# LANL-Bioinformatics/KWAGE

Measured on AMD Instinct MI355X. Metric: G k-mer·sample bit-tests/sec (+ achieved HBM GB/s of the gather kernel in `roofline`), higher is better.
Workload: dtype u32

## Files before the change

kwage_amd/csrc/engine.hip:

```cpp
#include <hip/hip_runtime.h>
#include <hip/hip_ext.h>

#include <algorithm>
#include <chrono>
#include <cmath>
#include <cstdio>
#include <cctype>
#include <cstring>
#include <new>
#include <string>
#include <thread>
#include <vector>

#include <unistd.h>

#include "host.hpp"
#include "engine_state.hpp"
#include "kernels.hpp"

using namespace kwage;


struct TuningName { const char *name; int64_t Tuning::*field; };
static const TuningName TUNING_NAMES[] = {
// ... 51 lines not shown

__global__ __launch_bounds__(256) void remap_rows_kernel(uint32_t *rows, const uint64_t *pos_off, const uint32_t *nkmer, uint32_t num_hash,
                                                         const uint32_t *map, uint32_t map_len, unsigned long long *missing, uint32_t wgs_per_query)
{
	const uint32_t q = blockIdx.x / wgs_per_query, part = blockIdx.x % wgs_per_query;
	uint32_t *rq = rows + pos_off[q]*num_hash;
	const uint64_t n = (uint64_t)nkmer[q]*num_hash;
	for(uint64_t e = (uint64_t)part*blockDim.x + threadIdx.x; e < n; e += (uint64_t)wgs_per_query*blockDim.x){
		const uint32_t r = rq[e];
		uint32_t lo = 0, hi = map_len;
		while(lo < hi){
			const uint32_t mid = lo + (hi - lo)/2;
			if(map[mid] < r){ lo = mid + 1; } else { hi = mid; }
		}
		if(lo < map_len && map[lo] == r){ rq[e] = lo; }
		else{ rq[e] = 0; atomicAdd(missing, 1ull); }
	}
}

__global__ __launch_bounds__(SEARCH_THREADS) void and_refine_emit_kernel(SearchArgs a, RefineArgs ra)
{
	constexpr int B = 4;
	__shared__ WaveHitBuf hit_bufs[SEARCH_THREADS/WAVE];
	WaveHitBuf *hbuf = &hit_bufs[threadIdx.x >> 6];
	WaveHitState hst;
	const uint32_t lane = threadIdx.x & (WAVE - 1), l = lane & 7u, g = lane >> 3;
	const uint32_t n_clusters = refine_list_end(ra, 0);
	const uint32_t gw = __builtin_amdgcn_readfirstlane(blockIdx.x*(blockDim.x/WAVE) + (threadIdx.x >> 6));
	const uint32_t nw = gridDim.x*(blockDim.x/WAVE);
	for(uint64_t c0 = gw; c0 < n_clusters; c0 += (uint64_t)B*nw){
		RefineCluster cl[B];
		u32x4 m[B];
#pragma unroll
		for(int k = 0; k < B; ++k){
			const uint64_t ci = c0 + (uint64_t)k*nw;
			cl[k].q = REFINE_NONE;
			if(ci < n_clusters){ cl[k] = ra.clusters[ci]; }
		}
#pragma unroll
		for(int k = 0; k < B; ++k){
			const uint32_t groups = cl[k].kstep_groups & 0xFFu;
			m[k] = (u32x4)(0u);
			if(cl[k].q != REFINE_NONE && ((groups >> g) & 1u)){
				const uint32_t it = cl[k].first_item + __popc(groups & ((1u << g) - 1u));
				m[k] = reinterpret_cast<const u32x4*>(ra.masks)[(uint64_t)it*8 + l];
			}
		}
#pragma unroll
		for(int k = 0; k < B; ++k){
			if(cl[k].q == REFINE_NONE){ continue; }
			const uint32_t kstep = cl[k].kstep_groups >> 8;
			emit_masked_hits_buffered(a, hbuf, hst, cl[k].q, kstep*WAVE + lane, m[k], cl[k].n, (uint64_t)cl[k].q*a.runs_per_query + kstep);
		}
	}
	wave_hits_flush(a, hbuf, hst);
}

__global__ __launch_bounds__(256) void band_bucket_kernel(const uint32_t *__restrict__ rows, const uint64_t *__restrict__ pos_off, const uint32_t *__restrict__ nkmer,
                                                         uint32_t num_hash, uint32_t bands, uint32_t rows_per_band, uint32_t *__restrict__ loc, uint32_t *__restrict__ rows2)
{
// ... 407 lines not shown
template <int PLANES>
int launch_count_combine(const SearchArgs &a, uint32_t seg_planes, hipStream_t s, const StageEvents &ge)
{
	const size_t lds = (size_t)(COMBINE_WAVES/2)*PLANES*WAVE*16;
	if(lds > 48*1024){
		HIP_TRY(hipFuncSetAttribute((const void*)count_combine_kernel<PLANES>, hipFuncAttributeMaxDynamicSharedMemorySize, (int)lds));
	}
	KW_GATHER_LAUNCH(ge, false, true, (count_combine_kernel<PLANES>), dim3((a.units_per_row + WAVE - 1)/WAVE, a.n_queries), dim3(COMBINE_WAVES*WAVE), lds, s, a, seg_planes);
	return KWAGE_OK;
}

uint64_t max_segments(const SearchArgs &a, uint64_t max_segs) { return (a.n_queries > 65535) ? 1 : max_segs; }

int reserve_zeroed(DevBuf &buf, uint64_t bytes, hipStream_t s)
{
	if(bytes <= buf.cap){ return KWAGE_OK; }
	int rc = buf.reserve(bytes);
	if(rc){ return rc; }
	HIP_TRY(hipMemsetAsync(buf.p, 0, buf.cap, s));
	return KWAGE_OK;
}

int refine_setup(Slot *sl, const Tuning &tn, const SearchArgs &a, uint64_t total_rows, uint64_t max_rows, uint32_t max_seg, uint64_t item_bytes, uint64_t unit_bytes,
                 uint64_t tiles, uint64_t screen_waves, uint64_t ncu, hipStream_t gs, RefineSetup *out,
                 uint64_t exact_clusters = 0, uint64_t exact_items = 0, uint64_t exact_units = 0)
{
	int rc;
	RefineArgs &ra = out->ra;
	ra.seg_rows = (uint32_t)std::min<int64_t>(std::max<int64_t>(tn.refine_seg_rows, 8), max_seg);
	ra.seg_rows = (uint32_t)std::max<uint64_t>(ra.seg_rows, (max_rows + 65535)/65536);
	ra.min_rows = (uint32_t)std::max<int64_t>(tn.refine_min_rows, 1);
	ra.max_groups = (uint32_t)std::min<int64_t>(std::max<int64_t>(tn.refine_max_groups, 0), 16);
	uint64_t items = std::min<uint64_t>(std::max<uint64_t>(8ull*a.n_queries, 1u << 16), 1u << 20);
	items = std::max<uint64_t>(std::min<uint64_t>(items, (256ull << 20)/item_bytes), 1024);
	uint64_t units = std::min<uint64_t>(std::max<uint64_t>(32*total_rows/ra.seg_rows, 1u << 18), 1u << 25);
	if(unit_bytes){ units = std::max<uint64_t>(std::min<uint64_t>(units, (512ull << 20)/unit_bytes), 4096); }
	if(tn.refine_list_cap > 0){ items = units = (uint64_t)std::min<int64_t>(tn.refine_list_cap, 1 << 20); }
	uint64_t clusters = items;
	if(exact_units){ clusters = exact_clusters; items = exact_items; units = exact_units; }
	if(exact_units && tn.refine_list_cap > 0){ clusters = items = units = (uint64_t)std::min<int64_t>(tn.refine_list_cap, 1 << 20); }
	const uint64_t tiles_per_wave = (tiles + screen_waves - 1)/std::max<uint64_t>(screen_waves, 1);
	auto list = [&](uint64_t cap, uint64_t stat_max, uint64_t chunk_max) {
		RefineList ls;
		ls.cap = (uint32_t)cap;
		ls.stat = (tn.refine_static && !exact_units) ? (uint32_t)std::min<uint64_t>(stat_max, cap/2/std::max<uint64_t>(screen_waves, 1)) : 0u;
		ls.base = (uint32_t)(ls.stat*screen_waves);
		ls.chunk = exact_units ? 1u : (uint32_t)std::max<uint64_t>(1, std::min<uint64_t>(chunk_max, tiles_per_wave/4));
		return ls;
	};
	ra.lc = list(clusters, 32, 32);
	ra.li = list(items, 64, 64);
	ra.lu = list(units, 256, 256);
	if((rc = sl->ref_counters.reserve(8*sizeof(uint32_t)))){ return rc; }
	if((rc = sl->ref_clusters.reserve(clusters*sizeof(RefineCluster)))){ return rc; }
	if((rc = sl->ref_masks.reserve(items*item_bytes))){ return rc; }
	if((rc = sl->ref_units.reserve(units*sizeof(RefineUnit)))){ return rc; }
	if(unit_bytes && (rc = sl->ref_slab.reserve(units*unit_bytes))){ return rc; }
	ra.counters = (uint32_t*)sl->ref_counters.p;
	ra.clusters = (RefineCluster*)sl->ref_clusters.p;
	ra.masks = (uint32_t*)sl->ref_masks.p;
	ra.units = (RefineUnit*)sl->ref_units.p;
	ra.slab = (uint32_t*)sl->ref_slab.p;
	HIP_TRY(hipMemsetAsync(ra.counters, 0, 8*sizeof(uint32_t), gs));
	sl->ref_base[0] = ra.lc.base; sl->ref_base[1] = ra.li.base; sl->ref_base[2] = ra.lu.base;
	sl->ref_cap[0] = ra.lc.cap; sl->ref_cap[1] = ra.li.cap; sl->ref_cap[2] = ra.lu.cap;
	ra.queue_batch = (uint32_t)std::max<uint64_t>(1, std::min<uint64_t>(16, tiles/(8*std::max<uint64_t>(screen_waves, 1))));
	ra.check_every = (tn.count_screen_check == 16 || tn.count_screen_check == 32 || tn.count_screen_check == 64) ? (uint32_t)tn.count_screen_check : 8u;
	out->refine_wgs = (uint32_t)(ncu*8);
	out->emit_wgs = (uint32_t)(ncu*4);
	return KWAGE_OK;
}

uint32_t count_screen_blocks_per_cu(uint32_t planes, uint32_t nh)
{
	static int cache[3][5] = {};
	const int pi = (planes <= 7) ? 0 : (planes <= 10) ? 1 : 2, ni = (int)std::min(std::max(nh, 1u), 5u) - 1;
	if(cache[pi][ni] == 0){
		int nb = 0;
		hipError_t e = hipErrorUnknown;
#define KWAGE_OCC_NH(P, N) case N: e = hipOccupancyMaxActiveBlocksPerMultiprocessor(&nb, count_screen_kernel<P, N>, SEARCH_THREADS, 0); break;
#define KWAGE_OCC_P(I, P) case I: switch(ni + 1){ KWAGE_OCC_NH(P, 1) KWAGE_OCC_NH(P, 2) KWAGE_OCC_NH(P, 3) KWAGE_OCC_NH(P, 4) default: KWAGE_OCC_NH(P, 5) } break;
		switch(pi){ KWAGE_OCC_P(0, 7) KWAGE_OCC_P(1, 10) default: KWAGE_OCC_P(2, 14) }
#undef KWAGE_OCC_P
#undef KWAGE_OCC_NH
		if(e != hipSuccess || nb <= 0){ (void)hipGetLastError(); nb = 2; }
		cache[pi][ni] = nb;
// ... 39 lines not shown
			const uint32_t G = (a.units_per_row <= 4) ? 16 : (a.units_per_row <= 8) ? 8 : (a.units_per_row <= 16) ? 4 : 2;
			const uint64_t waves = ((uint64_t)a.n_queries + G - 1)/G;
			const dim3 grid((uint32_t)((waves + 3)/4)), block(SEARCH_THREADS);
			const int unroll = (waves < ncu*16) ? 16 : 8;
			snprintf(sl->kernel_name, sizeof(sl->kernel_name), "and_narrow_kernel<%u,%d>", G, unroll);
#define KWAGE_NARROW_CASE(GG) case GG: \
				if(unroll == 16){ KW_GATHER_LAUNCH(ge, true, true, (and_narrow_kernel<GG, 16>), grid, block, 0, gs, a); } \
				else{ KW_GATHER_LAUNCH(ge, true, true, (and_narrow_kernel<GG, 8>), grid, block, 0, gs, a); } break;
			switch(G){
				KWAGE_NARROW_CASE(16) KWAGE_NARROW_CASE(8) KWAGE_NARROW_CASE(4)
				default: KWAGE_NARROW_CASE(2)
			}
#undef KWAGE_NARROW_CASE
			HIP_TRY(hipGetLastError());
			return KWAGE_OK;
		}
		if(a.early_exit && tn.ee_refine && a.units_per_row >= WAVE && tn.force_segs <= 0){
			RefineSetup rs;
			const int vec = (a.units_per_row >= 4*WAVE) ? 2 : 1;
			a.segs = 1;
			a.chunks = (a.units_per_row + WAVE*vec - 1)/(WAVE*vec);
			const uint64_t tiles = (uint64_t)a.n_queries*a.chunks;
			const uint64_t screen_waves = (std::min<uint64_t>(tiles, ncu*(uint64_t)std::max<int64_t>(tn.screen_wpc, 1)) + 3)/4*4;
			if((rc = refine_setup(sl, tn, a, L->total_pos*a.num_hash, L->max_pos*a.num_hash, 1u << 20, 128, 0, tiles, screen_waves, ncu, gs, &rs))){ return rc; }
			const int unroll = (tn.refine_unroll == 16) ? 16 : 8;
			snprintf(sl->kernel_name, sizeof(sl->kernel_name), "and_screen_kernel<%d,8>+refine<%d>", vec, unroll);
			const dim3 grid((uint32_t)(screen_waves/4)), block(SEARCH_THREADS);
			if(vec == 2){ KW_GATHER_LAUNCH(ge, true, false, (and_screen_kernel<2, 8>), grid, block, 0, gs, a, rs.ra); }
			else{ KW_GATHER_LAUNCH(ge, true, false, (and_screen_kernel<1, 8>), grid, block, 0, gs, a, rs.ra); }
			if(unroll == 16){ KW_GATHER_LAUNCH(ge, false, false, (and_refine_kernel<16>), dim3(rs.refine_wgs), block, 0, gs, a, rs.ra); }
			else{ KW_GATHER_LAUNCH(ge, false, false, (and_refine_kernel<8>), dim3(rs.refine_wgs), block, 0, gs, a, rs.ra); }
			KW_GATHER_LAUNCH(ge, false, true, and_refine_emit_kernel, dim3(rs.emit_wgs), block, 0, gs, a, rs.ra);
			HIP_TRY(hipGetLastError());
			return KWAGE_OK;
		}
		const int walk_knob = (int)tn.walk;
		const uint64_t walk_min_rows = (tn.walk_min_rows >= 0) ? (uint64_t)tn.walk_min_rows : (uint64_t)WALK_MIN_ROWS_PER_WAVE*256*WALK_WAVES_PER_CU;
		const uint32_t kib = (a.units_per_row + WAVE - 1)/WAVE;
		const uint32_t walk_max_kib = (uint32_t)std::max<int64_t>(tn.walk_max_kib, 0);
		const uint32_t walk_tile = (uint32_t)std::min<int64_t>(std::max<int64_t>(tn.walk_tile_kib, 1), 16);
		const uint32_t coltiles = (kib + walk_tile - 1)/walk_tile, walk_ch = (kib + coltiles - 1)/coltiles;
		const bool walk_ee_ok = !a.early_exit;
		const uint64_t walk_slots = (uint64_t)coltiles*L->total_pos;
		const uint32_t walk_min_kib = (uint32_t)std::max<int64_t>(tn.walk_min_kib, 1);
		const int walk_unroll = (walk_ch <= 2) ? 8 : 4;
		if(walk_knob && walk_ee_ok && kib >= walk_min_kib && kib <= walk_max_kib && walk_slots*a.num_hash >= walk_min_rows && walk_slots > 0){
			const uint64_t chip_waves = ncu*WALK_WAVES_PER_CU;
// ... 80 lines not shown
			HIP_TRY(hipMemsetAsync(sl->partial.p, 0xFF, bytes, gs));
			a.partial = (uint32_t*)sl->partial.p;
		}
		snprintf(sl->kernel_name, sizeof(sl->kernel_name), "and_kernel<%d,8,nt>%s", cfg.vec, a.segs > 1 ? "+segments" : "");
		launch_and_v(a, gs, cfg, ge);
		if(a.segs > 1){
			KW_GATHER_LAUNCH(ge, false, true, and_combine_kernel, dim3((a.units_per_row + 255)/256, a.n_queries), dim3(256), 0, gs, a);
		}
	}
	else{
		a.chunks = (a.units_per_row + WAVE - 1)/WAVE;
		const uint32_t planes = planes_for(L->max_pos);
		const bool narrow = tn.narrow && a.units_per_row <= 32 && a.units_per_row > 8 && a.n_queries >= 64 && planes <= 14;
		if(a.early_exit && tn.ee_refine && !narrow && tn.force_segs <= 0 && a.units_per_row >= WAVE
		   && (uint64_t)a.n_queries*a.chunks >= (uint64_t)std::max<int64_t>(tn.count_screen_min_tiles, 1) && planes <= 14){
			const uint64_t tiles = (uint64_t)a.n_queries*a.chunks;
			uint32_t seg = (uint32_t)std::min<int64_t>(std::max<int64_t>(tn.refine_seg_rows, 8), 120)/8*8;
			int up = 7;
			if(L->max_pos > 8192){ seg = (uint32_t)((L->max_pos + 127)/128 + 7)/8*8; up = 14; }
			const uint64_t wpc = std::min<uint64_t>((uint64_t)std::max<int64_t>(tn.count_screen_wpc, 1), 4ull*count_screen_blocks_per_cu(planes, std::min(a.num_hash, 5u)));
			const uint64_t screen_waves = (std::min<uint64_t>(tiles, ncu*wpc) + 3)/4*4;
			if((rc = check_refine_units(planes, up))){ return rc; }
			RefineSetup rs;
			if((rc = refine_setup(sl, tn, a, L->total_pos, 0, seg, (uint64_t)planes*128, (uint64_t)up*128, tiles, screen_waves, ncu, gs, &rs))){ return rc; }
			rs.ra.seg_rows = seg;
			a.segs = 1;
			snprintf(sl->kernel_name, sizeof(sl->kernel_name), "count_screen_kernel<%u,%u>+refine<%d>", planes, std::min(a.num_hash, 5u), up);
			const dim3 grid((uint32_t)(screen_waves/4)), block(SEARCH_THREADS);
#define KWAGE_CS_NH(P, N) case N: KW_GATHER_LAUNCH(ge, true, false, (count_screen_kernel<P, N>), grid, block, 0, gs, a, rs.ra); break;
#define KWAGE_CS_P(P) case P: switch(std::min(a.num_hash, 5u)){ KWAGE_CS_NH(P, 1) KWAGE_CS_NH(P, 2) KWAGE_CS_NH(P, 3) KWAGE_CS_NH(P, 4) default: KWAGE_CS_NH(P, 5) } break;
			switch(planes){ KWAGE_CS_P(7) KWAGE_CS_P(10) default: KWAGE_CS_P(14) }
#undef KWAGE_CS_P
#undef KWAGE_CS_NH
			launch_count_refine_and_emit(planes, up, a, rs, gs, ge);
			HIP_TRY(hipGetLastError());
			return KWAGE_OK;
		}
		if(a.early_exit && tn.ee_refine && tn.count_trunc && tn.count_walk && !narrow && tn.force_segs <= 0 && a.units_per_row >= WAVE && L->total_pos > 0){
			const uint32_t nq = a.n_queries;
			const uint32_t tplanes = std::max<uint32_t>(planes, 10);
			const double col = std::min(1.0, std::max(0.0, g->density_max) + 3.0*std::sqrt(0.25/4096.0));
			const double pm = std::min(0.9, std::max(0.0005, std::pow(col, (double)a.num_hash)));
			static const bool trunc_debug = getenv("KWAGE_TRUNC_DEBUG") != nullptr;
			if(trunc_debug){ fprintf(stderr, "[kwage_amd] truncated count walk: sampled density %.5f, densest column %.5f, per-k-mer match probability planned with %.5f\n", g->density, g->density_max, pm); }
			if((rc = sl->trunc_host.reserve(((uint64_t)nq + 1)*sizeof(uint64_t) + (uint64_t)nq*sizeof(uint32_t)))){ return rc; }
			uint64_t *h_soff = (uint64_t*)sl->trunc_host.p;
			uint32_t *h_kcut = (uint32_t*)(h_soff + nq + 1);
// ... 16 lines not shown
				max_rest = std::max(max_rest, npos - kc);
				rest_total += npos - kc;
			}
			const uint64_t slots = (uint64_t)a.chunks*walked;
			const uint64_t chip_waves = ncu*(uint64_t)std::max<int64_t>(tn.count_walk_wpc, 1);
			const uint64_t min_rows = (tn.count_walk_min_rows >= 0) ? (uint64_t)tn.count_walk_min_rows : (uint64_t)WALK_MIN_ROWS_PER_WAVE*chip_waves;
			uint64_t seg = (uint64_t)std::min<int64_t>(std::max<int64_t>(tn.refine_seg_rows, 8), 120)/8*8;
			seg = std::max<uint64_t>(seg, ((max_rest + 127)/128 + 7)/8*8);
			const int up = (seg <= 120) ? 7 : 14;
			uint64_t units_worst = 0;
			for(uint32_t i = 0; i < nq && seg; ++i){
				const uint64_t rest = (L->h_pos_off[i + 1] - L->h_pos_off[i]) - h_kcut[i];
				units_worst += (uint64_t)a.chunks*8*((rest + seg - 1)/seg);
			}
			const uint64_t tiles = (uint64_t)nq*a.chunks;
			const uint64_t units_cap = std::max<uint64_t>(4096, std::min<uint64_t>(units_worst, (1ull << 30)/((uint64_t)up*128 + sizeof(RefineUnit))));
			if(walked*10 <= L->total_pos*7 && slots*a.num_hash >= min_rows && seg <= 16376 && rest_total > 0 && tiles*8*(uint64_t)tplanes*128 <= (1ull << 30)){
				const uint64_t want_waves = (tn.count_walk_waves > 0) ? std::min<uint64_t>((uint64_t)tn.count_walk_waves, slots)
					: std::max<uint64_t>(1, std::min<uint64_t>(chip_waves, slots*a.num_hash/WALK_MIN_ROWS_PER_WAVE));
				const WalkShape shape = walk_shape(tn, want_waves, ncu);
				const uint64_t waves = (uint64_t)shape.wgs*shape.wg_waves;
				if((rc = check_refine_units(tplanes, up))){ return rc; }
				RefineSetup rs;
				if((rc = refine_setup(sl, tn, a, rest_total, 0, (uint32_t)seg, (uint64_t)tplanes*128, (uint64_t)up*128, tiles, waves, ncu, gs, &rs, tiles, tiles*8, units_cap))){ return rc; }
				rs.ra.seg_rows = (uint32_t)seg;
				if((rc = sl->trunc_dev.reserve(((uint64_t)nq + 1)*sizeof(uint64_t) + (uint64_t)nq*sizeof(uint32_t)))){ return rc; }
				HIP_TRY(hipMemcpyAsync(sl->trunc_dev.p, sl->trunc_host.p, ((uint64_t)nq + 1)*sizeof(uint64_t) + (uint64_t)nq*sizeof(uint32_t), hipMemcpyHostToDevice, gs));
				CountWalkArgs wa;
				wa.total_slots = slots;
				wa.per_wave = (slots + waves - 1)/waves;
				wa.coltiles = a.chunks;
				if((rc = sl->cwalk_slab.reserve(waves*2*tplanes*1024))){ return rc; }
				if((rc = reserve_zeroed(sl->cwalk_arrived, waves*CWALK_LEVELS*sizeof(uint32_t), gs))){ return rc; }
				wa.slab = (uint32_t*)sl->cwalk_slab.p;
				wa.arrived = (uint32_t*)sl->cwalk_arrived.p;
				wa.slot_off = (const uint64_t*)sl->trunc_dev.p;
				wa.kcut = (const uint32_t*)((const uint64_t*)sl->trunc_dev.p + nq + 1);
				a.segs = 1;
				snprintf(sl->kernel_name, sizeof(sl->kernel_name), "count_walk_kernel<%u,%u,trunc>+refine<%d>", tplanes, std::min(a.num_hash, 5u), up);
				launch_count_walk_planes<true>(tplanes, a, wa, rs.ra, shape, gs, ge);
				launch_count_refine_and_emit(tplanes, up, a, rs, gs, ge);
				HIP_TRY(hipGetLastError());
				return KWAGE_OK;
			}
		}
		if(tn.count_walk && !a.early_exit && !narrow && tn.force_segs <= 0 && L->total_pos > 0){
			const uint64_t slots = (uint64_t)a.chunks*L->total_pos;
// ... 296 lines not shown
			                   (const uint32_t*)bufs[j]->p, n, d + j);
		}
		e = hipGetLastError();
	}
	unsigned long long h[5] = {0, 0, 0, 0, 0};
	if(e == hipSuccess){ e = hipMemcpyAsync(h, d, sizeof(h), hipMemcpyDeviceToHost, ctx->stream); }
	if(e == hipSuccess){ e = hipStreamSynchronize(ctx->stream); }
	(void)hipFree(d);
	if(e != hipSuccess){ return fail(KWAGE_ERR_DEVICE, "kwage_ctx_scratch_nonzero: %s", hipGetErrorString(e)); }
	for(int j = 0; j < 5; ++j){ out[j] = h[j]; }
	return KWAGE_OK;
}

extern "C" int kwage_ctx_refine_stats(kwage_ctx *ctx, uint64_t out[8])
{
	if(!ctx || !out){ return fail(KWAGE_ERR_ARG, "kwage_ctx_refine_stats: NULL argument"); }
	for(int i = 0; i < 2; ++i){ if(ctx->slot[i].busy){ return fail(KWAGE_ERR_STATE, "kwage_ctx_refine_stats: a search is pending on this context"); } }
	int rc = set_device(ctx);
	if(rc){ return rc; }
	HIP_TRY(hipStreamSynchronize(ctx->gather_stream));
	for(int k = 0; k < 2; ++k){
		Slot *sl = &ctx->slot[k];
		uint32_t h[4] = {0, 0, 0, 0};
		if(sl->ref_counters.p){ HIP_TRY(hipMemcpy(h, sl->ref_counters.p, sizeof(h), hipMemcpyDeviceToHost)); }
		for(int j = 0; j < 3; ++j){ out[4*k + j] = std::min<uint64_t>((uint64_t)sl->ref_base[j] + h[j], sl->ref_cap[j]); }
		out[4*k + 3] = sl->ref_cap[2];
	}
	return KWAGE_OK;
}

namespace kwage {
hipStream_t ctx_stream(kwage_ctx *ctx) { return ctx->stream; }
int ctx_device(kwage_ctx *ctx) { return ctx->device; }
}

extern "C" int kwage_device_count(void)
{
	int n = 0;
	if(hipGetDeviceCount(&n) != hipSuccess){ return 0; }
	return n;
}

extern "C" int kwage_init(int device, kwage_ctx **out)
{
	if(!out){ return fail(KWAGE_ERR_ARG, "kwage_init: out is NULL"); }
	*out = nullptr;
	int n = 0;
	hipError_t e = hipGetDeviceCount(&n);
// ... 607 lines not shown
```

kwage_amd/csrc/engine_state.hpp:

```cpp
#ifndef KWAGE_AMD_ENGINE_STATE_HPP
#define KWAGE_AMD_ENGINE_STATE_HPP

#include <hip/hip_runtime.h>

#include <algorithm>
#include <deque>
#include <memory>
#include <mutex>
#include <vector>

#include "internal.h"

#define HIP_TRY(expr)                                                                          \
	do {                                                                                       \
		hipError_t _e = (expr);                                                                \
		if(_e != hipSuccess){                                                                  \
			return fail(KWAGE_ERR_DEVICE, "%s failed: %s (%s:%d)", #expr, hipGetErrorString(_e), \
			            __FILE__, __LINE__);                                                   \
		}                                                                                      \
	} while(0)

struct kwage_group;
struct kwage_batch;
struct kwage_ctx;
// ... 181 lines not shown
	uint32_t *d_nkmer = nullptr, *d_qthr = nullptr;
	kwage_hit *d_hits = nullptr;
	uint64_t hit_cap = 0, head_bytes = 0;
	PinBuf h_stage;
	DevBuf sort_scratch;
	DevBuf runs;
	uint64_t n_runs = 0;
	uint32_t runs_per_query = 0;
	bool busy = false;
	kwage_group *g = nullptr;
	kwage_batch *b = nullptr;
	const KmerLayout *lay = nullptr;
	float threshold = 1.0f;
	uint32_t flags = 0;
	uint32_t launches = 0;
	char kernel_name[64] = "";
	DevBuf walk_or, walk_done;
	DevBuf band_rows, band_loc, band_or, band_state;
	DevBuf cwalk_slab, cwalk_arrived;
	DevBuf ref_counters, ref_clusters, ref_masks, ref_units, ref_slab;
	DevBuf trunc_dev;
	PinBuf trunc_host;
	uint32_t ref_base[3] = {0, 0, 0}, ref_cap[3] = {0, 0, 0};
	uint64_t staged_hits = 0;
	kwage_hit *ext_hits = nullptr;
	uint64_t ext_cap = 0;
	uint64_t *ext_count = nullptr;
	bool append = false, append_reset = false;
	uint32_t col_base = 0;
};

struct Tuning {
	int64_t walk = 4;
	int64_t walk_min_rows = -1;
	int64_t walk_max_kib = 16;
	int64_t walk_tile_kib = 16;
	int64_t walk_min_kib = 2;
	int64_t walk_waves = 0;
	int64_t walk_one_wg_per_cu = 1;
	int64_t walk_bands = -1;
	int64_t walk_bands_min_gib = 48;
	int64_t and_vec = 0;
	int64_t and_wide_min_kib = 16;
	int64_t and_wide = 1;
	int64_t narrow = 1;
	int64_t force_segs = 0;
// ... 156 lines not shown
```

kwage_amd/csrc/kernels.hpp:

```cpp
#ifndef KWAGE_AMD_KERNELS_HPP
#define KWAGE_AMD_KERNELS_HPP

#include <hip/hip_runtime.h>
#include <stdint.h>

#include "kwage_amd.h"
#include "kmer_device.hpp"

namespace kwage {

static constexpr int WAVE = 64;
static constexpr int KM_THREADS = 256;
static constexpr uint32_t KM_LDS_SLOTS = 4096;
static constexpr uint32_t KM_CHUNK = 1024;
static constexpr uint64_t KM_EMPTY = ~0ull;
static constexpr int SEARCH_THREADS = 256;


__device__ __forceinline__ uint32_t table_log2(uint64_t npos)
{
	uint32_t lg = 6;
	while((1ull << lg) < 2*npos){ ++lg; }
	return lg;
}
// ... 382 lines not shown
		if(SEG){
			if(live[v]){
				uint32_t *m = a.partial + ((uint64_t)q*a.units_per_row + unit[v])*4;
#pragma unroll
				for(int d = 0; d < 4; ++d){
					if(acc[v][d] != ~0u){ atomicAnd(m + d, acc[v][d]); }
				}
			}
		}
		else{
			emit_mask_hits(a, q, unit[v], acc[v], n, (uint64_t)q*a.runs_per_query + c*VEC + v, live[v]);
		}
	}
}

struct RefineUnit { uint32_t item, r0, r1, unit0, rq_lo, rq_hi, q, pad; };
struct RefineCluster {
	uint32_t q, kstep_groups, first_item, n;
	uint32_t first_unit, nseg, pad0, pad1;
};
static constexpr uint32_t REFINE_NONE = 0xFFFFFFFFu;

struct RefineList { uint32_t cap, stat, base, chunk; };
struct RefineArgs {
	uint32_t *counters;
	RefineCluster *clusters;
	uint32_t *masks;
	RefineUnit *units;
	uint32_t *slab;
	RefineList lc, li, lu;
	uint32_t seg_rows;
	uint32_t min_rows;
	uint32_t max_groups;
	uint32_t queue_batch;
	uint32_t check_every;
};

__device__ __forceinline__ uint32_t group_bits(uint64_t lanes)
{
	uint32_t g = 0;
#pragma unroll
	for(int k = 0; k < 8; ++k){ g |= ((lanes >> (8*k)) & 0xFFull) ? (1u << k) : 0u; }
	return g;
}

__device__ __forceinline__ uint32_t nth_set_bit(uint32_t bits, uint32_t j)
{
	for(uint32_t k = 0; k < j; ++k){ bits &= bits - 1; }
	return __ffs(bits) - 1;
}

struct RefineChunk { uint32_t next = 0, end = 0; };

__device__ __forceinline__ void refine_none_clusters(const RefineArgs &ra, uint32_t from, uint32_t to)
{
	to = min(to, ra.lc.cap);
	for(uint32_t i = from + (threadIdx.x & (WAVE - 1)); i < to; i += WAVE){ ra.clusters[i].q = REFINE_NONE; }
}
__device__ __forceinline__ void refine_none_units(const RefineArgs &ra, uint32_t from, uint32_t to)
{
	to = min(to, ra.lu.cap);
	for(uint32_t i = from + (threadIdx.x & (WAVE - 1)); i < to; i += WAVE){ ra.units[i].item = REFINE_NONE; }
}

__device__ __forceinline__ uint32_t refine_take(const RefineArgs &ra, int which, RefineChunk &ch, uint32_t need)
{
	const RefineList &ls = (which == 0) ? ra.lc : (which == 1) ? ra.li : ra.lu;
	if(ch.end - ch.next < need){
		if(which == 0){ refine_none_clusters(ra, ch.next, ch.end); } else if(which == 2){ refine_none_units(ra, ch.next, ch.end); }
		ch.next = ch.end = 0;
		if((uint64_t)ls.base + __hip_atomic_load(ra.counters + which, __ATOMIC_RELAXED, __HIP_MEMORY_SCOPE_AGENT) >= ls.cap){ return REFINE_NONE; }
		const uint32_t want = max(need, ls.chunk);
		uint32_t r = 0;
		if((threadIdx.x & (WAVE - 1)) == 0){ r = atomicAdd(ra.counters + which, want); }
		const uint64_t at = (uint64_t)ls.base + __builtin_amdgcn_readfirstlane(r);
		if(at + want > ls.cap){
			if(at < ls.cap){
				if(which == 0){ refine_none_clusters(ra, (uint32_t)at, ls.cap); } else if(which == 2){ refine_none_units(ra, (uint32_t)at, ls.cap); }
			}
			return REFINE_NONE;
		}
		ch.next = (uint32_t)at;
		ch.end = (uint32_t)at + want;
	}
	const uint32_t at = ch.next;
	ch.next += need;
	return at;
}

__device__ __forceinline__ uint32_t refine_list_end(const RefineArgs &ra, int which)
{
	const RefineList &ls = (which == 0) ? ra.lc : (which == 1) ? ra.li : ra.lu;
	return (uint32_t)min((uint64_t)ls.base + ra.counters[which], (uint64_t)ls.cap);
}

template <int VEC, int UNROLL>
__global__ __launch_bounds__(SEARCH_THREADS) void and_screen_kernel(SearchArgs a, RefineArgs ra)
{
	const uint32_t lane = threadIdx.x & (WAVE - 1);
	const uint64_t n_tiles = (uint64_t)a.n_queries*a.chunks;
	const uint32_t n_waves = gridDim.x*(blockDim.x/WAVE);
	const uint32_t gw = __builtin_amdgcn_readfirstlane(blockIdx.x*(blockDim.x/WAVE) + (threadIdx.x >> 6));
	__shared__ WaveHitBuf hit_bufs[SEARCH_THREADS/WAVE];
	WaveHitBuf *hbuf = &hit_bufs[threadIdx.x >> 6];
	WaveHitState hst;
	RefineChunk cc, ci, cu;
	cc.next = gw*ra.lc.stat; cc.end = cc.next + ra.lc.stat;
	ci.next = gw*ra.li.stat; ci.end = ci.next + ra.li.stat;
	cu.next = gw*ra.lu.stat; cu.end = cu.next + ra.lu.stat;
	bool lists_full = false;
	for(uint64_t tile = gw; tile < n_tiles; tile += n_waves){
		const uint32_t q = __builtin_amdgcn_readfirstlane((uint32_t)(tile / a.chunks));
		const uint32_t c = __builtin_amdgcn_readfirstlane((uint32_t)(tile % a.chunks));
		const uint32_t n = a.nkmer[q];
		if(n == 0){ continue; }
		const uint32_t nrows = n*a.num_hash;
		const uint64_t rq_off = a.pos_off[q]*a.num_hash;
		const uint32_t *rq = a.rows + rq_off;

		uint32_t unit[VEC];
		u32x4 acc[VEC];
#pragma unroll
		for(int v = 0; v < VEC; ++v){
			const uint32_t u = c*(WAVE*VEC) + v*WAVE + lane;
			const bool live = (u < a.units_per_row);
			unit[v] = live ? u : (a.units_per_row - 1);
			acc[v] = live ? reinterpret_cast<const u32x4*>(a.valid)[u] : (u32x4)(0u);
		}

		bool may_hand_over = !lists_full, gone = false;
		uint32_t i = 0;
		for(; i + UNROLL <= nrows; i += UNROLL){
// ... 5 lines not shown
#pragma unroll
				for(int v = 0; v < VEC; ++v){ x[u][v] = load16<true>(p + unit[v]); }
			}
#pragma unroll
			for(int u = 0; u < UNROLL; ++u){
#pragma unroll
				for(int v = 0; v < VEC; ++v){ acc[v] &= x[u][v]; }
			}
			uint32_t gb[VEC], ngroups = 0;
#pragma unroll
			for(int v = 0; v < VEC; ++v){
				gb[v] = group_bits(__ballot((acc[v].x | acc[v].y | acc[v].z | acc[v].w) != 0));
				ngroups += __popc(gb[v]);
			}
			if(ngroups == 0){ gone = true; break; }
			const uint32_t done = i + UNROLL;
			if(may_hand_over && ngroups <= ra.max_groups && nrows - done >= ra.min_rows && (done >= 2*UNROLL || nrows < 4*ra.seg_rows)){
				may_hand_over = false;
				const uint32_t nseg = (nrows - done + ra.seg_rows - 1)/ra.seg_rows;
				uint32_t nc = 0;
#pragma unroll
				for(int v = 0; v < VEC; ++v){ nc += gb[v] ? 1u : 0u; }
				const uint32_t nu = ngroups*nseg;
				const uint32_t c0 = refine_take(ra, 0, cc, nc);
				const uint32_t i0 = (c0 != REFINE_NONE) ? refine_take(ra, 1, ci, ngroups) : REFINE_NONE;
				const uint32_t u0 = (i0 != REFINE_NONE) ? refine_take(ra, 2, cu, nu) : REFINE_NONE;
				if(u0 == REFINE_NONE){
					if(c0 != REFINE_NONE){ refine_none_clusters(ra, c0, c0 + nc); }
					lists_full = true;
					continue;
				}
				uint32_t cidx = c0, ii = i0, all_groups = 0;
#pragma unroll
				for(int v = 0; v < VEC; ++v){
					all_groups |= gb[v] << (8*v);
					if(!gb[v]){ continue; }
					if(lane == 0){
						RefineCluster cl; cl.q = q; cl.kstep_groups = ((c*VEC + v) << 8) | gb[v]; cl.first_item = ii; cl.n = n;
						cl.first_unit = 0; cl.nseg = 0; cl.pad0 = 0; cl.pad1 = 0;
						ra.clusters[cidx] = cl;
					}
					const uint32_t k = lane >> 3;
					if((gb[v] >> k) & 1u){
						const uint32_t it = ii + __popc(gb[v] & ((1u << k) - 1u));
						reinterpret_cast<u32x4*>(ra.masks)[(uint64_t)it*8 + (lane & 7u)] = acc[v];
					}
					++cidx;
					ii += __popc(gb[v]);
				}
// ... 6 lines not shown
					un.r1 = min(nrows, un.r0 + ra.seg_rows);
					un.unit0 = c*(WAVE*VEC) + gpos*8u;
					un.rq_lo = (uint32_t)rq_off; un.rq_hi = (uint32_t)(rq_off >> 32);
					un.q = q; un.pad = 0;
					ra.units[u0 + e] = un;
				}
				gone = true;
				break;
			}
		}
		if(gone){ continue; }
		for(; i < nrows; ++i){
			const uint32_t r = rq[i];
			const u32x4 *p = reinterpret_cast<const u32x4*>(a.db + (uint64_t)r*a.stride);
#pragma unroll
			for(int v = 0; v < VEC; ++v){ acc[v] &= load16<true>(p + unit[v]); }
		}
#pragma unroll
		for(int v = 0; v < VEC; ++v){
			emit_masked_hits_buffered(a, hbuf, hst, q, unit[v], acc[v], n, (uint64_t)q*a.runs_per_query + c*VEC + v);
		}
	}
	wave_hits_flush(a, hbuf, hst);
	refine_none_clusters(ra, cc.next, cc.end);
	refine_none_units(ra, cu.next, cu.end);
}

template <int UNROLL>
__global__ __launch_bounds__(SEARCH_THREADS) void and_refine_kernel(SearchArgs a, RefineArgs ra)
{
	static_assert(UNROLL == 8 || UNROLL == 16, "eight or sixteen rows in flight");
	const uint32_t lane = threadIdx.x & (WAVE - 1), l = lane & 7u, sh = lane & ~7u;
	const uint32_t n_units = refine_list_end(ra, 2);
	const uint64_t gw = (uint64_t)blockIdx.x*(blockDim.x/WAVE) + (threadIdx.x >> 6);
	const uint64_t step = (uint64_t)gridDim.x*(blockDim.x/WAVE)*8;
	for(uint64_t base = gw*8; base < n_units; base += step){
		const uint64_t u = base + (lane >> 3);
		RefineUnit un;
		un.item = REFINE_NONE;
		if(u < n_units){ un = ra.units[u]; }
		bool on = (un.item != REFINE_NONE);
		uint32_t *M = ra.masks;
		u32x4 m = (u32x4)(0u);
		if(on){
			M = ra.masks + ((uint64_t)un.item*8 + l)*4;
#pragma unroll
			for(int d = 0; d < 4; ++d){ m[d] = __hip_atomic_load(M + d, __ATOMIC_RELAXED, __HIP_MEMORY_SCOPE_AGENT); }
		}
		on = on && (((uint32_t)(__ballot((m.x | m.y | m.z | m.w) != 0) >> sh) & 0xFFu) != 0);
		if(on){
			const uint32_t *rq = a.rows + (((uint64_t)un.rq_hi << 32) | un.rq_lo);
			const u32x4 *col = reinterpret_cast<const u32x4*>(a.db) + (un.unit0 + l);
			u32x4 acc = ~(u32x4)(0u);
			bool alive = true;
			for(uint32_t b = un.r0; alive && b < un.r1; b += 64){
				uint32_t idx[8];
#pragma unroll
				for(int k = 0; k < 8; ++k){ idx[k] = rq[min(b + 8u*k + l, un.r1 - 1)]; }
#pragma unroll
				for(int k = 0; k < 8; k += UNROLL/8){
					if(b + 8u*k >= un.r1){ break; }
					u32x4 x[UNROLL];
#pragma unroll
					for(int j = 0; j < UNROLL; ++j){
						const uint32_t r = __shfl(idx[k + j/8], sh + (j & 7));
						x[j] = load16<true>(reinterpret_cast<const u32x4*>(reinterpret_cast<const uint8_t*>(col) + (uint64_t)r*a.stride));
					}
#pragma unroll
					for(int j = 0; j < UNROLL; ++j){ acc &= x[j]; }
					if((((uint32_t)(__ballot((acc.x | acc.y | acc.z | acc.w) != 0) >> sh)) & 0xFFu) == 0){ alive = false; break; }
				}
			}
#pragma unroll
			for(int d = 0; d < 4; ++d){
				if(m[d] & ~acc[d]){ __hip_atomic_fetch_and(M + d, acc[d], __ATOMIC_RELAXED, __HIP_MEMORY_SCOPE_AGENT); }
			}
		}
	}
}


static constexpr int WALK_WG_WAVES = 8;
static constexpr uint32_t WALK_DEAD = 1u;
static constexpr uint32_t WALK_DIRTY = 2u;

struct WalkArgs {
	uint64_t total_slots;
	uint64_t per_wave;
	uint32_t coltiles;
	uint32_t *orbuf;
// ... 1031 lines not shown
```

Baseline: 52310.

## Compact static refine lists via prefix sums and double-buffer refine counters

Screen waves now record how many entries of their static cluster and unit slots they used, instead of filling the unused slots with REFINE_NONE sentinels. The refine and emit kernels build an LDS prefix sum over these per-wave counts, so they walk only live entries, and the emit kernel gives each wave a contiguous range. The refine counters are double-buffered and the next set is zeroed inside the screen kernel, which removes a per-call memset. The refine kernel also issues the first row-index loads before the mask check and adds a sched_barrier to group its gathers. In exchange, each block runs a 5120-entry prefix scan over 20 KB of LDS, which may lower occupancy.

```diff
diff --git a/kwage_amd/csrc/engine.hip b/kwage_amd/csrc/engine.hip
--- a/kwage_amd/csrc/engine.hip
+++ b/kwage_amd/csrc/engine.hip
@@ -97,20 +97,35 @@
 {
 	constexpr int B = 4;
 	__shared__ WaveHitBuf hit_bufs[SEARCH_THREADS/WAVE];
+	__shared__ uint32_t pre[REFINE_STAT_WAVES];
 	WaveHitBuf *hbuf = &hit_bufs[threadIdx.x >> 6];
 	WaveHitState hst;
 	const uint32_t lane = threadIdx.x & (WAVE - 1), l = lane & 7u, g = lane >> 3;
-	const uint32_t n_clusters = refine_list_end(ra, 0);
+	const uint32_t n_dyn = refine_list_end(ra, 0) - ra.lc.base;
+	const uint32_t n_stat = refine_dense_prefix<0>(ra, pre);
+	const uint64_t n_clusters = (uint64_t)n_stat + n_dyn;
 	const uint32_t gw = __builtin_amdgcn_readfirstlane(blockIdx.x*(blockDim.x/WAVE) + (threadIdx.x >> 6));
 	const uint32_t nw = gridDim.x*(blockDim.x/WAVE);
-	for(uint64_t c0 = gw; c0 < n_clusters; c0 += (uint64_t)B*nw){
+	const uint64_t per = (n_clusters + (uint64_t)B*nw - 1)/((uint64_t)B*nw)*B;
+	const uint64_t c_end = min(n_clusters, (gw + 1)*per);
+	uint32_t w = 0, lo = 0, hi = 0;
+	if(gw*per < n_stat){
+		w = refine_dense_wave(ra, pre, (uint32_t)(gw*per));
+		lo = pre[w];
+		hi = (w + 1 < ra.stat_waves) ? pre[w + 1] : n_stat;
+	}
+	for(uint64_t c0 = gw*per; c0 < c_end; c0 += B){
 		RefineCluster cl[B];
 		u32x4 m[B];
 #pragma unroll
 		for(int k = 0; k < B; ++k){
-			const uint64_t ci = c0 + (uint64_t)k*nw;
+			const uint64_t ci = c0 + k;
 			cl[k].q = REFINE_NONE;
-			if(ci < n_clusters){ cl[k] = ra.clusters[ci]; }
+			if(ci < n_stat){
+				while((uint32_t)ci >= hi){ ++w; lo = hi; hi = (w + 1 < ra.stat_waves) ? pre[w + 1] : n_stat; }
+				cl[k] = ra.clusters[w*ra.lc.stat + ((uint32_t)ci - lo)];
+			}
+			else if(ci < c_end){ cl[k] = ra.clusters[ra.lc.base + (uint32_t)(ci - n_stat)]; }
 		}
 #pragma unroll
 		for(int k = 0; k < B; ++k){
@@ -564,7 +579,7 @@
 }
 
 int refine_setup(Slot *sl, const Tuning &tn, const SearchArgs &a, uint64_t total_rows, uint64_t max_rows, uint32_t max_seg, uint64_t item_bytes, uint64_t unit_bytes,
-                 uint64_t tiles, uint64_t screen_waves, uint64_t ncu, hipStream_t gs, RefineSetup *out,
+                 uint64_t tiles, uint64_t screen_waves, uint64_t ncu, hipStream_t gs, bool dense, RefineSetup *out,
                  uint64_t exact_clusters = 0, uint64_t exact_items = 0, uint64_t exact_units = 0)
 {
 	int rc;
@@ -582,28 +597,35 @@
 	if(exact_units){ clusters = exact_clusters; items = exact_items; units = exact_units; }
 	if(exact_units && tn.refine_list_cap > 0){ clusters = items = units = (uint64_t)std::min<int64_t>(tn.refine_list_cap, 1 << 20); }
 	const uint64_t tiles_per_wave = (tiles + screen_waves - 1)/std::max<uint64_t>(screen_waves, 1);
+	const uint64_t stat_waves = dense ? std::min<uint64_t>(screen_waves, REFINE_STAT_WAVES) : screen_waves;
 	auto list = [&](uint64_t cap, uint64_t stat_max, uint64_t chunk_max) {
 		RefineList ls;
 		ls.cap = (uint32_t)cap;
 		ls.stat = (tn.refine_static && !exact_units) ? (uint32_t)std::min<uint64_t>(stat_max, cap/2/std::max<uint64_t>(screen_waves, 1)) : 0u;
-		ls.base = (uint32_t)(ls.stat*screen_waves);
+		ls.base = (uint32_t)(ls.stat*stat_waves);
 		ls.chunk = exact_units ? 1u : (uint32_t)std::max<uint64_t>(1, std::min<uint64_t>(chunk_max, tiles_per_wave/4));
 		return ls;
 	};
 	ra.lc = list(clusters, 32, 32);
 	ra.li = list(items, 64, 64);
 	ra.lu = list(units, 256, 256);
-	if((rc = sl->ref_counters.reserve(8*sizeof(uint32_t)))){ return rc; }
+	if((rc = reserve_zeroed(sl->ref_counters, (16 + REFINE_STAT_WAVES)*sizeof(uint32_t), gs))){ return rc; }
 	if((rc = sl->ref_clusters.reserve(clusters*sizeof(RefineCluster)))){ return rc; }
 	if((rc = sl->ref_masks.reserve(items*item_bytes))){ return rc; }
 	if((rc = sl->ref_units.reserve(units*sizeof(RefineUnit)))){ return rc; }
 	if(unit_bytes && (rc = sl->ref_slab.reserve(units*unit_bytes))){ return rc; }
-	ra.counters = (uint32_t*)sl->ref_counters.p;
+	sl->ref_block ^= 1u;
+	sl->ref_dense = dense;
+	ra.counters = (uint32_t*)sl->ref_counters.p + 8*sl->ref_block;
+	ra.counters_next = (uint32_t*)sl->ref_counters.p + 8*(sl->ref_block ^ 1u);
+	ra.used = (uint32_t*)sl->ref_counters.p + 16;
+	ra.stat_waves = dense ? (uint32_t)stat_waves : 0u;
 	ra.clusters = (RefineCluster*)sl->ref_clusters.p;
 	ra.masks = (uint32_t*)sl->ref_masks.p;
 	ra.units = (RefineUnit*)sl->ref_units.p;
 	ra.slab = (uint32_t*)sl->ref_slab.p;
-	HIP_TRY(hipMemsetAsync(ra.counters, 0, 8*sizeof(uint32_t), gs));
+	if(!dense){ HIP_TRY(hipMemsetAsync(sl->ref_counters.p, 0, 16*sizeof(uint32_t), gs)); }
+	sl->ref_stat_waves = ra.stat_waves;
 	sl->ref_base[0] = ra.lc.base; sl->ref_base[1] = ra.li.base; sl->ref_base[2] = ra.lu.base;
 	sl->ref_cap[0] = ra.lc.cap; sl->ref_cap[1] = ra.li.cap; sl->ref_cap[2] = ra.lu.cap;
 	ra.queue_batch = (uint32_t)std::max<uint64_t>(1, std::min<uint64_t>(16, tiles/(8*std::max<uint64_t>(screen_waves, 1))));
@@ -689,7 +711,7 @@
 			a.chunks = (a.units_per_row + WAVE*vec - 1)/(WAVE*vec);
 			const uint64_t tiles = (uint64_t)a.n_queries*a.chunks;
 			const uint64_t screen_waves = (std::min<uint64_t>(tiles, ncu*(uint64_t)std::max<int64_t>(tn.screen_wpc, 1)) + 3)/4*4;
-			if((rc = refine_setup(sl, tn, a, L->total_pos*a.num_hash, L->max_pos*a.num_hash, 1u << 20, 128, 0, tiles, screen_waves, ncu, gs, &rs))){ return rc; }
+			if((rc = refine_setup(sl, tn, a, L->total_pos*a.num_hash, L->max_pos*a.num_hash, 1u << 20, 128, 0, tiles, screen_waves, ncu, gs, true, &rs))){ return rc; }
 			const int unroll = (tn.refine_unroll == 16) ? 16 : 8;
 			snprintf(sl->kernel_name, sizeof(sl->kernel_name), "and_screen_kernel<%d,8>+refine<%d>", vec, unroll);
 			const dim3 grid((uint32_t)(screen_waves/4)), block(SEARCH_THREADS);
@@ -816,7 +838,7 @@
 			const uint64_t screen_waves = (std::min<uint64_t>(tiles, ncu*wpc) + 3)/4*4;
 			if((rc = check_refine_units(planes, up))){ return rc; }
 			RefineSetup rs;
-			if((rc = refine_setup(sl, tn, a, L->total_pos, 0, seg, (uint64_t)planes*128, (uint64_t)up*128, tiles, screen_waves, ncu, gs, &rs))){ return rc; }
+			if((rc = refine_setup(sl, tn, a, L->total_pos, 0, seg, (uint64_t)planes*128, (uint64_t)up*128, tiles, screen_waves, ncu, gs, false, &rs))){ return rc; }
 			rs.ra.seg_rows = seg;
 			a.segs = 1;
 			snprintf(sl->kernel_name, sizeof(sl->kernel_name), "count_screen_kernel<%u,%u>+refine<%d>", planes, std::min(a.num_hash, 5u), up);
@@ -879,7 +901,7 @@
 				const uint64_t waves = (uint64_t)shape.wgs*shape.wg_waves;
 				if((rc = check_refine_units(tplanes, up))){ return rc; }
 				RefineSetup rs;
-				if((rc = refine_setup(sl, tn, a, rest_total, 0, (uint32_t)seg, (uint64_t)tplanes*128, (uint64_t)up*128, tiles, waves, ncu, gs, &rs, tiles, tiles*8, units_cap))){ return rc; }
+				if((rc = refine_setup(sl, tn, a, rest_total, 0, (uint32_t)seg, (uint64_t)tplanes*128, (uint64_t)up*128, tiles, waves, ncu, gs, false, &rs, tiles, tiles*8, units_cap))){ return rc; }
 				rs.ra.seg_rows = (uint32_t)seg;
 				if((rc = sl->trunc_dev.reserve(((uint64_t)nq + 1)*sizeof(uint64_t) + (uint64_t)nq*sizeof(uint32_t)))){ return rc; }
 				HIP_TRY(hipMemcpyAsync(sl->trunc_dev.p, sl->trunc_host.p, ((uint64_t)nq + 1)*sizeof(uint64_t) + (uint64_t)nq*sizeof(uint32_t), hipMemcpyHostToDevice, gs));
@@ -1222,8 +1244,16 @@
 	for(int k = 0; k < 2; ++k){
 		Slot *sl = &ctx->slot[k];
 		uint32_t h[4] = {0, 0, 0, 0};
-		if(sl->ref_counters.p){ HIP_TRY(hipMemcpy(h, sl->ref_counters.p, sizeof(h), hipMemcpyDeviceToHost)); }
+		if(sl->ref_counters.p){ HIP_TRY(hipMemcpy(h, (const uint32_t*)sl->ref_counters.p + 8*sl->ref_block, sizeof(h), hipMemcpyDeviceToHost)); }
 		for(int j = 0; j < 3; ++j){ out[4*k + j] = std::min<uint64_t>((uint64_t)sl->ref_base[j] + h[j], sl->ref_cap[j]); }
+		if(sl->ref_dense && sl->ref_counters.p){
+			std::vector<uint32_t> used(REFINE_STAT_WAVES);
+			HIP_TRY(hipMemcpy(used.data(), (const uint32_t*)sl->ref_counters.p + 16, used.size()*sizeof(uint32_t), hipMemcpyDeviceToHost));
+			uint64_t uc = 0, uu = 0;
+			for(uint32_t w = 0; w < sl->ref_stat_waves; ++w){ uc += used[w] & 0xFFFFu; uu += used[w] >> 16; }
+			out[4*k + 0] = out[4*k + 0] - sl->ref_base[0] + uc;
+			out[4*k + 2] = out[4*k + 2] - sl->ref_base[2] + uu;
+		}
 		out[4*k + 3] = sl->ref_cap[2];
 	}
 	return KWAGE_OK;
diff --git a/kwage_amd/csrc/engine_state.hpp b/kwage_amd/csrc/engine_state.hpp
--- a/kwage_amd/csrc/engine_state.hpp
+++ b/kwage_amd/csrc/engine_state.hpp
@@ -227,6 +227,8 @@
 	DevBuf trunc_dev;
 	PinBuf trunc_host;
 	uint32_t ref_base[3] = {0, 0, 0}, ref_cap[3] = {0, 0, 0};
+	uint32_t ref_block = 0, ref_stat_waves = 0;
+	bool ref_dense = false;
 	uint64_t staged_hits = 0;
 	kwage_hit *ext_hits = nullptr;
 	uint64_t ext_cap = 0;
diff --git a/kwage_amd/csrc/kernels.hpp b/kwage_amd/csrc/kernels.hpp
--- a/kwage_amd/csrc/kernels.hpp
+++ b/kwage_amd/csrc/kernels.hpp
@@ -428,8 +428,12 @@
 static constexpr uint32_t REFINE_NONE = 0xFFFFFFFFu;
 
 struct RefineList { uint32_t cap, stat, base, chunk; };
+static constexpr uint32_t REFINE_STAT_WAVES = 5120;
 struct RefineArgs {
 	uint32_t *counters;
+	uint32_t *counters_next;
+	uint32_t *used;
+	uint32_t stat_waves;
 	RefineCluster *clusters;
 	uint32_t *masks;
 	RefineUnit *units;
@@ -456,7 +460,7 @@
 	return __ffs(bits) - 1;
 }
 
-struct RefineChunk { uint32_t next = 0, end = 0; };
+struct RefineChunk { uint32_t next = 0, end = 0, first = 0, used = 0; bool stat = false; };
 
 __device__ __forceinline__ void refine_none_clusters(const RefineArgs &ra, uint32_t from, uint32_t to)
 {
@@ -469,11 +473,13 @@
 	for(uint32_t i = from + (threadIdx.x & (WAVE - 1)); i < to; i += WAVE){ ra.units[i].item = REFINE_NONE; }
 }
 
+template <bool DENSE = false>
 __device__ __forceinline__ uint32_t refine_take(const RefineArgs &ra, int which, RefineChunk &ch, uint32_t need)
 {
 	const RefineList &ls = (which == 0) ? ra.lc : (which == 1) ? ra.li : ra.lu;
 	if(ch.end - ch.next < need){
-		if(which == 0){ refine_none_clusters(ra, ch.next, ch.end); } else if(which == 2){ refine_none_units(ra, ch.next, ch.end); }
+		if(DENSE && ch.stat){ ch.used = ch.next - ch.first; ch.stat = false; }
+		else if(which == 0){ refine_none_clusters(ra, ch.next, ch.end); } else if(which == 2){ refine_none_units(ra, ch.next, ch.end); }
 		ch.next = ch.end = 0;
 		if((uint64_t)ls.base + __hip_atomic_load(ra.counters + which, __ATOMIC_RELAXED, __HIP_MEMORY_SCOPE_AGENT) >= ls.cap){ return REFINE_NONE; }
 		const uint32_t want = max(need, ls.chunk);
@@ -500,6 +506,63 @@
 	return (uint32_t)min((uint64_t)ls.base + ra.counters[which], (uint64_t)ls.cap);
 }
 
+template <int WHICH>
+__device__ __forceinline__ uint32_t refine_dense_prefix(const RefineArgs &ra, uint32_t *pre)
+{
+	constexpr uint32_t PER = REFINE_STAT_WAVES/SEARCH_THREADS;
+	static_assert(REFINE_STAT_WAVES % (4*SEARCH_THREADS) == 0 && SEARCH_THREADS/WAVE <= 4, "whole 16-byte loads per thread; the waves' sums fit pre[0..3]");
+	const uint32_t lane = threadIdx.x & (WAVE - 1), wv = threadIdx.x >> 6, w0 = threadIdx.x*PER;
+	uint32_t c[PER], sum = 0;
+	u32x4 v[PER/4];
+#pragma unroll
+	for(uint32_t k = 0; k < PER/4; ++k){ v[k] = (u32x4)(0u); }
+	if(w0 < ra.stat_waves){
+#pragma unroll
+		for(uint32_t k = 0; k < PER/4; ++k){ v[k] = *reinterpret_cast<const u32x4*>(ra.used + w0 + 4*k); }
+	}
+#pragma unroll
+	for(uint32_t k = 0; k < PER; k += 4){
+		if(w0 + k >= ra.stat_waves){ v[k/4] = (u32x4)(0u); }
+#pragma unroll
+		for(int d = 0; d < 4; ++d){ c[k + d] = (WHICH == 0) ? (v[k/4][d] & 0xFFFFu) : (v[k/4][d] >> 16); sum += c[k + d]; }
+	}
+	uint32_t inc = sum;
+#pragma unroll
+	for(uint32_t d = 1; d < WAVE; d <<= 1){
+		const uint32_t o = __shfl_up(inc, d);
+		if(lane >= d){ inc += o; }
+	}
+	if(lane == WAVE - 1){ pre[wv] = inc; }
+	__syncthreads();
+	uint32_t off = inc - sum, total = 0;
+#pragma unroll
+	for(uint32_t w = 0; w < SEARCH_THREADS/WAVE; ++w){
+		const uint32_t s = pre[w];
+		if(w < wv){ off += s; }
+		total += s;
+	}
+	__syncthreads();
+#pragma unroll
+	for(uint32_t k = 0; k < PER; ++k){ pre[w0 + k] = off; off += c[k]; }
+	__syncthreads();
+	return total;
+}
+
+__device__ __forceinline__ uint32_t refine_dense_wave(const RefineArgs &ra, const uint32_t *pre, uint32_t d)
+{
+	uint32_t lo = 0, n = ra.stat_waves;
+	while(n > 0){
+		const uint32_t half = n/2;
+		if(pre[lo + half] <= d){ lo += half + 1; n -= half + 1; } else { n = half; }
+	}
+	return lo - 1;
+}
+__device__ __forceinline__ uint32_t refine_dense_place(const RefineArgs &ra, const uint32_t *pre, uint32_t d, uint32_t stat)
+{
+	const uint32_t w = refine_dense_wave(ra, pre, d);
+	return w*stat + (d - pre[w]);
+}
+
 template <int VEC, int UNROLL>
 __global__ __launch_bounds__(SEARCH_THREADS) void and_screen_kernel(SearchArgs a, RefineArgs ra)
 {
@@ -511,9 +574,12 @@
 	WaveHitBuf *hbuf = &hit_bufs[threadIdx.x >> 6];
 	WaveHitState hst;
 	RefineChunk cc, ci, cu;
-	cc.next = gw*ra.lc.stat; cc.end = cc.next + ra.lc.stat;
-	ci.next = gw*ra.li.stat; ci.end = ci.next + ra.li.stat;
-	cu.next = gw*ra.lu.stat; cu.end = cu.next + ra.lu.stat;
+	if(gw < ra.stat_waves){
+		cc.first = cc.next = gw*ra.lc.stat; cc.end = cc.next + ra.lc.stat; cc.stat = true;
+		ci.first = ci.next = gw*ra.li.stat; ci.end = ci.next + ra.li.stat;
+		cu.first = cu.next = gw*ra.lu.stat; cu.end = cu.next + ra.lu.stat; cu.stat = true;
+	}
+	if(blockIdx.x == 0 && threadIdx.x < 8){ ra.counters_next[threadIdx.x] = 0; }
 	bool lists_full = false;
 	for(uint64_t tile = gw; tile < n_tiles; tile += n_waves){
 		const uint32_t q = __builtin_amdgcn_readfirstlane((uint32_t)(tile / a.chunks));
@@ -565,9 +631,9 @@
 #pragma unroll
 				for(int v = 0; v < VEC; ++v){ nc += gb[v] ? 1u : 0u; }
 				const uint32_t nu = ngroups*nseg;
-				const uint32_t c0 = refine_take(ra, 0, cc, nc);
-				const uint32_t i0 = (c0 != REFINE_NONE) ? refine_take(ra, 1, ci, ngroups) : REFINE_NONE;
-				const uint32_t u0 = (i0 != REFINE_NONE) ? refine_take(ra, 2, cu, nu) : REFINE_NONE;
+				const uint32_t c0 = refine_take<true>(ra, 0, cc, nc);
+				const uint32_t i0 = (c0 != REFINE_NONE) ? refine_take<true>(ra, 1, ci, ngroups) : REFINE_NONE;
+				const uint32_t u0 = (i0 != REFINE_NONE) ? refine_take<true>(ra, 2, cu, nu) : REFINE_NONE;
 				if(u0 == REFINE_NONE){
 					if(c0 != REFINE_NONE){ refine_none_clusters(ra, c0, c0 + nc); }
 					lists_full = true;
@@ -620,41 +686,55 @@
 		}
 	}
 	wave_hits_flush(a, hbuf, hst);
-	refine_none_clusters(ra, cc.next, cc.end);
-	refine_none_units(ra, cu.next, cu.end);
+	const uint32_t used_c = cc.stat ? cc.next - cc.first : cc.used, used_u = cu.stat ? cu.next - cu.first : cu.used;
+	if(gw < ra.stat_waves && lane == 0){ ra.used[gw] = (used_u << 16) | used_c; }
+	if(!cc.stat){ refine_none_clusters(ra, cc.next, cc.end); }
+	if(!cu.stat){ refine_none_units(ra, cu.next, cu.end); }
 }
 
 template <int UNROLL>
 __global__ __launch_bounds__(SEARCH_THREADS) void and_refine_kernel(SearchArgs a, RefineArgs ra)
 {
 	static_assert(UNROLL == 8 || UNROLL == 16, "eight or sixteen rows in flight");
+	__shared__ uint32_t pre[REFINE_STAT_WAVES];
 	const uint32_t lane = threadIdx.x & (WAVE - 1), l = lane & 7u, sh = lane & ~7u;
-	const uint32_t n_units = refine_list_end(ra, 2);
+	const uint32_t n_dyn = refine_list_end(ra, 2) - ra.lu.base;
+	const uint32_t n_stat = refine_dense_prefix<2>(ra, pre);
+	const uint64_t n_units = (uint64_t)n_stat + n_dyn;
 	const uint64_t gw = (uint64_t)blockIdx.x*(blockDim.x/WAVE) + (threadIdx.x >> 6);
 	const uint64_t step = (uint64_t)gridDim.x*(blockDim.x/WAVE)*8;
 	for(uint64_t base = gw*8; base < n_units; base += step){
 		const uint64_t u = base + (lane >> 3);
 		RefineUnit un;
 		un.item = REFINE_NONE;
-		if(u < n_units){ un = ra.units[u]; }
+		if(u < n_units){ un = ra.units[(u < n_stat) ? refine_dense_place(ra, pre, (uint32_t)u, ra.lu.stat) : ra.lu.base + (uint32_t)(u - n_stat)]; }
 		bool on = (un.item != REFINE_NONE);
 		uint32_t *M = ra.masks;
+		const uint32_t *rq = a.rows;
 		u32x4 m = (u32x4)(0u);
+		uint32_t idx[8];
+#pragma unroll
+		for(int k = 0; k < 8; ++k){ idx[k] = 0; }
 		if(on){
 			M = ra.masks + ((uint64_t)un.item*8 + l)*4;
+			rq = a.rows + (((uint64_t)un.rq_hi << 32) | un.rq_lo);
+#pragma unroll
+			for(int k = 0; k < 8; ++k){ idx[k] = rq[min(un.r0 + 8u*k + l, un.r1 - 1)]; }
 #pragma unroll
 			for(int d = 0; d < 4; ++d){ m[d] = __hip_atomic_load(M + d, __ATOMIC_RELAXED, __HIP_MEMORY_SCOPE_AGENT); }
+			asm volatile("" : "+v"(idx[0]), "+v"(idx[1]), "+v"(idx[2]), "+v"(idx[3]), "+v"(idx[4]), "+v"(idx[5]), "+v"(idx[6]), "+v"(idx[7]));
 		}
 		on = on && (((uint32_t)(__ballot((m.x | m.y | m.z | m.w) != 0) >> sh) & 0xFFu) != 0);
 		if(on){
-			const uint32_t *rq = a.rows + (((uint64_t)un.rq_hi << 32) | un.rq_lo);
 			const u32x4 *col = reinterpret_cast<const u32x4*>(a.db) + (un.unit0 + l);
 			u32x4 acc = ~(u32x4)(0u);
 			bool alive = true;
 			for(uint32_t b = un.r0; alive && b < un.r1; b += 64){
-				uint32_t idx[8];
-#pragma unroll
-				for(int k = 0; k < 8; ++k){ idx[k] = rq[min(b + 8u*k + l, un.r1 - 1)]; }
+				if(b != un.r0){
+#pragma unroll
+					for(int k = 0; k < 8; ++k){ idx[k] = rq[min(b + 8u*k + l, un.r1 - 1)]; }
+					asm volatile("" : "+v"(idx[0]), "+v"(idx[1]), "+v"(idx[2]), "+v"(idx[3]), "+v"(idx[4]), "+v"(idx[5]), "+v"(idx[6]), "+v"(idx[7]));
+				}
 #pragma unroll
 				for(int k = 0; k < 8; k += UNROLL/8){
 					if(b + 8u*k >= un.r1){ break; }
@@ -664,6 +744,7 @@
 						const uint32_t r = __shfl(idx[k + j/8], sh + (j & 7));
 						x[j] = load16<true>(reinterpret_cast<const u32x4*>(reinterpret_cast<const uint8_t*>(col) + (uint64_t)r*a.stride));
 					}
+					__builtin_amdgcn_sched_barrier(0);
 #pragma unroll
 					for(int j = 0; j < UNROLL; ++j){ acc &= x[j]; }
 					if((((uint32_t)(__ballot((acc.x | acc.y | acc.z | acc.w) != 0) >> sh)) & 0xFFu) == 0){ alive = false; break; }
```

Measured after the change: 52290 (median of 2 runs). Within noise of the previous version (-0.0%).
